# daxiongpro/EPNet

Hardware: AMD Instinct MI355X
Metric: SA-stack points/sec per GPU (16384-pt KITTI scene) + % HBM roofline (higher is better)
Workload: dtype f32; 1 GPU; 256 x 16384-pt kitti scenes per GPU per step through the 4-level SA op stack (4 samplings [FPS + centre gather; levels 2-4 nested in level 1 where tie-free] + 8 ball_query + 8 fused groupings [xyz - centre ; features]), pyramid 16384>4096>1024>256>64, radii [[.1,.5],[.5,1],[1,2],[2,4]], nsample [16,32], C=0/96/256/512, HIP-graph launch; levels=4, scenes_per_gpu=256, software_pipelined=True, pipeline_stages=2, parallelism=scene-parallel x1

## Files before the change

epnet_amd/csrc/group.hip:

```cpp

#include "common.h"
#include "spatial.h"
#include "runsum.h"

namespace epnet {

constexpr int kGThreads = 256;
constexpr int kGChan = 16;

__global__ __launch_bounds__(kGThreads) void gather_rows_vec4_kernel(int c, int n, int p, size_t ostride,
                                                                     const float *__restrict__ points,
                                                                     const int *__restrict__ idx,
                                                                     float *__restrict__ out) {
    int wg_x, wg_y, bs;
    xcd_scene_map3(wg_x, wg_y, bs);
    const int c0 = wg_y * kGChan;
    const int q4 = wg_x * kGThreads + threadIdx.x;
    if (q4 * 4 >= p) return;
    const int4 id = *reinterpret_cast<const int4 *>(idx + (size_t)bs * p + (size_t)q4 * 4);
    const int cend = min(c, c0 + kGChan);
    const float *src = points + ((size_t)bs * c + c0) * n;
    float *dst = out + (size_t)bs * ostride + (size_t)c0 * p + (size_t)q4 * 4;
#pragma unroll 4
    for (int ci = c0; ci < cend; ++ci) {
        float4 v;
        v.x = src[id.x];
        v.y = src[id.y];
        v.z = src[id.z];
        v.w = src[id.w];
        *reinterpret_cast<float4 *>(dst) = v;
        src += n;
        dst += p;
    }
}

__global__ __launch_bounds__(kGThreads) void gather_rows_scalar_kernel(int c, int n, int p, size_t ostride,
                                                                       const float *__restrict__ points,
                                                                       const int *__restrict__ idx,
                                                                       float *__restrict__ out) {
    int wg_x, wg_y, bs;
    xcd_scene_map3(wg_x, wg_y, bs);
    const int c0 = wg_y * kGChan;
    const int q = wg_x * kGThreads + threadIdx.x;
    if (q >= p) return;
    const int id = idx[(size_t)bs * p + q];
    const int cend = min(c, c0 + kGChan);
    for (int ci = c0; ci < cend; ++ci)
        out[(size_t)bs * ostride + (size_t)ci * p + q] = points[((size_t)bs * c + ci) * n + id];
}

#ifndef EPNET_GATHER_STAGE_UNROLL
#define EPNET_STAGE_PRAGMA
#else
#define EPNET_STAGE_STR2(x) #x
#define EPNET_STAGE_STR(x) EPNET_STAGE_STR2(unroll x)
#define EPNET_STAGE_PRAGMA _Pragma(EPNET_STAGE_STR(EPNET_GATHER_STAGE_UNROLL))
#endif
#ifndef EPNET_GATHER_LDS_BUDGET_KB
#define EPNET_GATHER_LDS_BUDGET_KB 64
#endif
#ifndef EPNET_GATHER_LDS_THREADS
#define EPNET_GATHER_LDS_THREADS 256
#endif
#ifndef EPNET_GATHER_LDS_UNROLL
#define EPNET_GATHER_LDS_UNROLL 1
#endif
constexpr int kGLdsThreads = EPNET_GATHER_LDS_THREADS;
__device__ __forceinline__ void stage_quads(const float *__restrict__ src, int groups, int n, float4 *__restrict__ s_quad,
                                            int threads) {
    const int n4 = n >> 2;
    for (int e = threadIdx.x; e < groups * n4; e += threads) {
        const int g = e / n4, j4 = e - g * n4;
        const float4 *row = reinterpret_cast<const float4 *>(src + (size_t)g * 4 * n) + j4;
        const float4 a = row[0], b4 = row[n4], cc = row[2 * n4], d = row[3 * n4];
        float4 *dst = s_quad + (size_t)g * n + j4 * 4;
        dst[0] = make_float4(a.x, b4.x, cc.x, d.x);
        dst[1] = make_float4(a.y, b4.y, cc.y, d.y);
        dst[2] = make_float4(a.z, b4.z, cc.z, d.z);
        dst[3] = make_float4(a.w, b4.w, cc.w, d.w);
    }
}

__device__ __forceinline__ void serve_quads(const float4 *__restrict__ quad, int groups, int n, int4 id, float *__restrict__ dst,
                                            int p) {
#pragma unroll 1
    for (int g = 0; g < groups; ++g) {
        const float4 v0 = quad[id.x], v1 = quad[id.y], v2 = quad[id.z], v3 = quad[id.w];
        store_stream(dst, v0.x, v1.x, v2.x, v3.x);
        store_stream(dst + p, v0.y, v1.y, v2.y, v3.y);
        store_stream(dst + 2 * (size_t)p, v0.z, v1.z, v2.z, v3.z);
        store_stream(dst + 3 * (size_t)p, v0.w, v1.w, v2.w, v3.w);
        quad += n;
        dst += 4 * (size_t)p;
    }
}

template <bool QUAD>
__global__ __launch_bounds__(kGLdsThreads) void gather_rows_lds_kernel(int c, int n, int p, int rows, int tile, size_t ostride,
                                                                    const float *__restrict__ points,
                                                                    const int *__restrict__ idx,
                                                                    float *__restrict__ out) {
    extern __shared__ float s_rows[];
    int wg_x, wg_y, bs;
    xcd_scene_map3(wg_x, wg_y, bs);
    const int c0 = wg_y * rows;
    const int nr = min(rows, c - c0);
    const float *src = points + ((size_t)bs * c + c0) * n;
    const int total = nr * n;
    if (QUAD) {
        stage_quads(src, nr >> 2, n, reinterpret_cast<float4 *>(s_rows), kGLdsThreads);
    } else if ((n & 3) == 0 && ((uintptr_t)src & 15) == 0) {
        const float4 *src4 = reinterpret_cast<const float4 *>(src);
        float4 *dst4 = reinterpret_cast<float4 *>(s_rows);
        EPNET_STAGE_PRAGMA
        for (int e = threadIdx.x; e < total / 4; e += kGLdsThreads) dst4[e] = src4[e];
    } else {
        for (int e = threadIdx.x; e < total; e += kGLdsThreads) s_rows[e] = src[e];
    }
    __syncthreads();
    const int q_begin = wg_x * tile, q_end = min(p, q_begin + tile);
    const int *ix = idx + (size_t)bs * p;
    float *dst_base = out + (size_t)bs * ostride + (size_t)c0 * p;
    for (int q = q_begin + threadIdx.x * 4; q < q_end; q += kGLdsThreads * 4) {
        const int4 id = *reinterpret_cast<const int4 *>(ix + q);
        float *dst = dst_base + q;
        if (QUAD) {
            serve_quads(reinterpret_cast<const float4 *>(s_rows), nr >> 2, n, id, dst, p);
            continue;
        }
        const float *row = s_rows;
#pragma unroll EPNET_GATHER_LDS_UNROLL
        for (int r = 0; r < nr; ++r) {
            float4 v;
            v.x = row[id.x];
            v.y = row[id.y];
            v.z = row[id.z];
            v.w = row[id.w];
            store_stream(dst, v.x, v.y, v.z, v.w);
            row += n;
            dst += p;
        }
    }
}

#ifndef EPNET_GATHER_LDS2_UNROLL
#define EPNET_GATHER_LDS2_UNROLL 1
#endif
constexpr long long kGatherLds2MinPositions = 3 * kGLdsThreads * 4;
template <bool QUAD>
__global__ __launch_bounds__(kGLdsThreads) void gather_rows_lds2_kernel(int c, int n, int rows, const float *__restrict__ points,
                                                                        int p0, size_t ostride0, const int *__restrict__ idx0,
                                                                        float *__restrict__ out0, int p1, size_t ostride1,
                                                                        const int *__restrict__ idx1, float *__restrict__ out1) {
    extern __shared__ float s_rows[];
    int wg_x, bs;
    xcd_scene_map(wg_x, bs);
    const int c0 = wg_x * rows;
    const int nr = min(rows, c - c0);
    const float *src = points + ((size_t)bs * c + c0) * n;
    const int total = nr * n;
    if (QUAD) {
        stage_quads(src, nr >> 2, n, reinterpret_cast<float4 *>(s_rows), kGLdsThreads);
    } else if ((n & 3) == 0 && ((uintptr_t)src & 15) == 0) {
        const float4 *src4 = reinterpret_cast<const float4 *>(src);
        float4 *dst4 = reinterpret_cast<float4 *>(s_rows);
        EPNET_STAGE_PRAGMA
        for (int e = threadIdx.x; e < total / 4; e += kGLdsThreads) dst4[e] = src4[e];
    } else {
        for (int e = threadIdx.x; e < total; e += kGLdsThreads) s_rows[e] = src[e];
    }
    __syncthreads();
#pragma unroll 1
    for (int set = 0; set < 2; ++set) {
        const int p = set ? p1 : p0;
        const int *ix = (set ? idx1 : idx0) + (size_t)bs * p;
        float *dst_base = (set ? out1 : out0) + (size_t)bs * (set ? ostride1 : ostride0) + (size_t)c0 * p;
        for (int q = threadIdx.x * 4; q < p; q += kGLdsThreads * 4) {
            const int4 id = *reinterpret_cast<const int4 *>(ix + q);
            float *dst = dst_base + q;
            if (QUAD) {
                serve_quads(reinterpret_cast<const float4 *>(s_rows), nr >> 2, n, id, dst, p);
                continue;
            }
            const float *row = s_rows;
#pragma unroll EPNET_GATHER_LDS2_UNROLL
            for (int r = 0; r < nr; ++r) {
                float4 v;
                v.x = row[id.x];
                v.y = row[id.y];
                v.z = row[id.z];
                v.w = row[id.w];
                store_stream(dst, v.x, v.y, v.z, v.w);
                row += n;
                dst += p;
            }
        }
    }
}

__global__ __launch_bounds__(kGThreads) void scatter_rows_lds_kernel(int c, int n, int p, int rows, size_t gstride,
                                                                     const float *__restrict__ grad_out,
                                                                     const int *__restrict__ idx,
                                                                     float *__restrict__ grad_points) {
    extern __shared__ float acc[];
    const int bs = blockIdx.y;
    const int c0 = blockIdx.x * rows;
    const int nr = min(rows, c - c0);
    for (int e = threadIdx.x; e < nr * n; e += kGThreads) acc[e] = 0.f;
    __syncthreads();
    const int *ix = idx + (size_t)bs * p;
    const float *go = grad_out + (size_t)bs * gstride + (size_t)c0 * p;
    for (int q = threadIdx.x; q < p; q += kGThreads) {
        const int id = ix[q];
        for (int r = 0; r < nr; ++r) atomicAdd(&acc[r * n + id], go[(size_t)r * p + q]);
    }
    __syncthreads();
    float *gp = grad_points + ((size_t)bs * c + c0) * n;
    for (int e = threadIdx.x; e < nr * n; e += kGThreads) gp[e] += acc[e];
}

__global__ __launch_bounds__(kGThreads) void scatter_rows_atomic_kernel(int c, int n, int p, size_t gstride,
                                                                        const float *__restrict__ grad_out,
                                                                        const int *__restrict__ idx,
                                                                        float *__restrict__ grad_points) {
    const int bs = blockIdx.z, ci = blockIdx.y;
    const int q = blockIdx.x * kGThreads + threadIdx.x;
    if (q >= p) return;
    atomicAdd(grad_points + ((size_t)bs * c + ci) * n + idx[(size_t)bs * p + q],
              grad_out[(size_t)bs * gstride + (size_t)ci * p + q]);
}

__global__ __launch_bounds__(kGThreads) void group_xyz_centred_kernel(int n, int npoints, int nsample, size_t ostride,
                                                                      const float *__restrict__ xyz,
                                                                      const float *__restrict__ new_xyz,
                                                                      const int *__restrict__ idx, float *__restrict__ out) {
    int wg_x, bs;
    xcd_scene_map(wg_x, bs);
    const int p = npoints * nsample;
    const int q = wg_x * kGThreads + threadIdx.x;
    if (q >= p) return;
    const int id = idx[(size_t)bs * p + q];
    const int ci = q / nsample;
    const float *pt = xyz + ((size_t)bs * n + id) * 3;
    const float *ce = new_xyz + ((size_t)bs * npoints + ci) * 3;
    float *dst = out + (size_t)bs * ostride + q;
    dst[0] = pt[0] - ce[0];
    dst[(size_t)p] = pt[1] - ce[1];
    dst[(size_t)p * 2] = pt[2] - ce[2];
}

__global__ __launch_bounds__(kGThreads) void group_xyz_centred_vec4_kernel(int n, int npoints, int nsample, size_t ostride,
                                                                           const float *__restrict__ xyz,
                                                                           const float *__restrict__ new_xyz,
                                                                           const int *__restrict__ idx,
                                                                           float *__restrict__ out) {
    int wg_x, bs;
    xcd_scene_map(wg_x, bs);
    const int p = npoints * nsample;
    const int q = (wg_x * kGThreads + threadIdx.x) * 4;
    if (q >= p) return;
    const int4 id = *reinterpret_cast<const int4 *>(idx + (size_t)bs * p + q);
    const float *base = xyz + (size_t)bs * n * 3;
    const float *ce = new_xyz + ((size_t)bs * npoints + q / nsample) * 3;
    const float cx = ce[0], cy = ce[1], cz = ce[2];
    const float *p0 = base + (size_t)id.x * 3, *p1 = base + (size_t)id.y * 3, *p2 = base + (size_t)id.z * 3,
                *p3 = base + (size_t)id.w * 3;
    float *dst = out + (size_t)bs * ostride + q;
    *reinterpret_cast<float4 *>(dst) = make_float4(p0[0] - cx, p1[0] - cx, p2[0] - cx, p3[0] - cx);
    *reinterpret_cast<float4 *>(dst + (size_t)p) = make_float4(p0[1] - cy, p1[1] - cy, p2[1] - cy, p3[1] - cy);
    *reinterpret_cast<float4 *>(dst + (size_t)p * 2) = make_float4(p0[2] - cz, p1[2] - cz, p2[2] - cz, p3[2] - cz);
}

__global__ __launch_bounds__(kGLdsThreads) void group_linear_lds_kernel(int c, int n, int npoints, int nsample, int rows, int tile,
                                                                        const float *__restrict__ z, const float *__restrict__ xyz,
                                                                        const float *__restrict__ new_xyz, const int *__restrict__ idx,
                                                                        const float *__restrict__ wx, const float *__restrict__ bias,
                                                                        float *__restrict__ out) {
    extern __shared__ float s_rows[];
    const int bs = blockIdx.z;
    const int c0 = blockIdx.y * rows;
    const int nr = min(rows, c - c0);
    const int p = npoints * nsample;
    const float *src = z + ((size_t)bs * c + c0) * n;
    const int total = nr * n;
    if ((n & 3) == 0 && ((uintptr_t)src & 15) == 0) {
        const float4 *src4 = reinterpret_cast<const float4 *>(src);
        float4 *dst4 = reinterpret_cast<float4 *>(s_rows);
        EPNET_STAGE_PRAGMA
        for (int e = threadIdx.x; e < total / 4; e += kGLdsThreads) dst4[e] = src4[e];
    } else {
        for (int e = threadIdx.x; e < total; e += kGLdsThreads) s_rows[e] = src[e];
    }
    __syncthreads();
    const int q_begin = blockIdx.x * tile, q_end = min(p, q_begin + tile);
    const int *ix = idx + (size_t)bs * p;
    const float *pts = xyz + (size_t)bs * n * 3;
    float *dst_base = out + ((size_t)bs * c + c0) * p;
    for (int q = q_begin + threadIdx.x * 4; q < q_end; q += kGLdsThreads * 4) {
        const int4 id = *reinterpret_cast<const int4 *>(ix + q);
        const float *ce = new_xyz + ((size_t)bs * npoints + q / nsample) * 3;
        const float cx = ce[0], cy = ce[1], cz = ce[2];
        const float *p0 = pts + (size_t)id.x * 3, *p1 = pts + (size_t)id.y * 3, *p2 = pts + (size_t)id.z * 3, *p3 = pts + (size_t)id.w * 3;
        const float dx0 = p0[0] - cx, dy0 = p0[1] - cy, dz0 = p0[2] - cz;
        const float dx1 = p1[0] - cx, dy1 = p1[1] - cy, dz1 = p1[2] - cz;
        const float dx2 = p2[0] - cx, dy2 = p2[1] - cy, dz2 = p2[2] - cz;
        const float dx3 = p3[0] - cx, dy3 = p3[1] - cy, dz3 = p3[2] - cz;
        float *dst = dst_base + q;
        const float *row = s_rows;
#pragma unroll 2
        for (int r = 0; r < nr; ++r) {
            const float w0 = wx[(c0 + r) * 3], w1 = wx[(c0 + r) * 3 + 1], w2 = wx[(c0 + r) * 3 + 2];
            float4 v;
            v.x = row[id.x] + (w0 * dx0 + w1 * dy0 + w2 * dz0);
            v.y = row[id.y] + (w0 * dx1 + w1 * dy1 + w2 * dz1);
            v.z = row[id.z] + (w0 * dx2 + w1 * dy2 + w2 * dz2);
            v.w = row[id.w] + (w0 * dx3 + w1 * dy3 + w2 * dz3);
            if (bias) {
                const float bv = bias[c0 + r];
                v.x += bv; v.y += bv; v.z += bv; v.w += bv;
            }
            store_stream(dst, v.x, v.y, v.z, v.w);
            row += n;
            dst += p;
        }
    }
}

__global__ __launch_bounds__(kGThreads) void group_linear_scalar_kernel(int c, int n, int npoints, int nsample,
                                                                        const float *__restrict__ z, const float *__restrict__ xyz,
                                                                        const float *__restrict__ new_xyz, const int *__restrict__ idx,
                                                                        const float *__restrict__ wx, const float *__restrict__ bias,
                                                                        float *__restrict__ out) {
    const int bs = blockIdx.z;
    const int c0 = blockIdx.y * kGChan;
    const int p = npoints * nsample;
    const int q = blockIdx.x * kGThreads + threadIdx.x;
    if (q >= p) return;
    const int id = idx[(size_t)bs * p + q];
    const float *pt = xyz + ((size_t)bs * n + id) * 3;
    const float *ce = new_xyz + ((size_t)bs * npoints + q / nsample) * 3;
    const float dx = pt[0] - ce[0], dy = pt[1] - ce[1], dz = pt[2] - ce[2];
    const int cend = min(c, c0 + kGChan);
    for (int ci = c0; ci < cend; ++ci) {
        float v = z[((size_t)bs * c + ci) * n + id] + (wx[ci * 3] * dx + wx[ci * 3 + 1] * dy + wx[ci * 3 + 2] * dz);
        if (bias) v += bias[ci];
        out[((size_t)bs * c + ci) * p + q] = v;
    }
}

constexpr int kGwRows = 8;
__global__ __launch_bounds__(kGThreads) void group_linear_grad_w_kernel(int c, int n, int npoints, int nsample, int tile,
                                                                        const float *__restrict__ grad_out,
                                                                        const float *__restrict__ xyz,
                                                                        const float *__restrict__ new_xyz,
                                                                        const int *__restrict__ idx, float *__restrict__ grad_w) {
    __shared__ float s_part[kGThreads / 64][kGwRows * 3];
    const int bs = blockIdx.z;
    const int c0 = blockIdx.y * kGwRows;
    const int nr = min(kGwRows, c - c0);
    const int p = npoints * nsample;
    const int q_begin = blockIdx.x * tile, q_end = min(p, q_begin + tile);
    const int *ix = idx + (size_t)bs * p;
    const float *pts = xyz + (size_t)bs * n * 3;
    const float *g = grad_out + ((size_t)bs * c + c0) * p;
    float acc[kGwRows][3];
#pragma unroll
    for (int r = 0; r < kGwRows; ++r) acc[r][0] = acc[r][1] = acc[r][2] = 0.f;
    for (int q = q_begin + threadIdx.x; q < q_end; q += kGThreads) {
        const int id = ix[q];
        const float *pt = pts + (size_t)id * 3;
        const float *ce = new_xyz + ((size_t)bs * npoints + q / nsample) * 3;
        float gv[kGwRows];
#pragma unroll
        for (int r = 0; r < kGwRows; ++r) gv[r] = g[(size_t)min(r, nr - 1) * p + q];
        const float dx = pt[0] - ce[0], dy = pt[1] - ce[1], dz = pt[2] - ce[2];
#pragma unroll
        for (int r = 0; r < kGwRows; ++r) {
            const float gr = r < nr ? gv[r] : 0.f;
            acc[r][0] += gr * dx;
            acc[r][1] += gr * dy;
            acc[r][2] += gr * dz;
        }
    }
    const int lane = lane_id(), wave = threadIdx.x >> 6;
#pragma unroll
    for (int r = 0; r < kGwRows; ++r)
#pragma unroll
        for (int k = 0; k < 3; ++k) {
            const float v = wave_sum_f32(acc[r][k]);
            if (lane == 0) s_part[wave][r * 3 + k] = v;
        }
    __syncthreads();
    if (threadIdx.x < nr * 3) {
        float v = 0.f;
#pragma unroll
        for (int w = 0; w < kGThreads / 64; ++w) v += s_part[w][threadIdx.x];
        atomicAdd(grad_w + (size_t)c0 * 3 + threadIdx.x, v);
    }
}

constexpr int kPmThreads = 256;
constexpr int kPmTile = 128;

__global__ __launch_bounds__(256) void transpose_cn_kernel(int c, int n, const float *__restrict__ src, float *__restrict__ dst) {
    __shared__ float tile[64][65];
    const int bs = blockIdx.z, n0 = blockIdx.x * 64, c0 = blockIdx.y * 64;
    src += (size_t)bs * c * n;
    dst += (size_t)bs * c * n;
    const int tx = threadIdx.x & 63, ty = threadIdx.x >> 6;
    for (int r = ty; r < 64; r += 4)
        if (c0 + r < c && n0 + tx < n) tile[r][tx] = src[(size_t)(c0 + r) * n + n0 + tx];
    __syncthreads();
    for (int r = ty; r < 64; r += 4)
        if (n0 + r < n && c0 + tx < c) dst[(size_t)(n0 + r) * c + c0 + tx] = tile[tx][r];
}

__device__ __forceinline__ int pm_slot(int ch, int r) { return ch * kPmTile + (r ^ (((ch >> 2) & 7) << 2)); }

__global__ __launch_bounds__(kPmThreads) void gather_rows_pm_kernel(int c, int n, int p, size_t ostride,
                                                                    const float *__restrict__ points_t,
                                                                    const int *__restrict__ idx, float *__restrict__ out) {
    extern __shared__ float s_tile[];
    int wg_x, bs;
    xcd_scene_map(wg_x, bs);
    const int q0 = wg_x * kPmTile;
    const int t = threadIdx.x, lane = t & 63, wave = t >> 6;
    const int lanes_per_row = c >> 2, rows_per_pass = kPmThreads / lanes_per_row;
    points_t += (size_t)bs * n * c;
    idx += (size_t)bs * p;
    out += (size_t)bs * ostride;
    const int cnt = min(kPmTile, p - q0);
    const int r_in = t / lanes_per_row, l_in = t - r_in * lanes_per_row;
    constexpr int kMaxPass = 8;
    if (r_in < rows_per_pass) {
        for (int r0 = r_in; r0 < cnt; r0 += rows_per_pass * kMaxPass) {
            int j[kMaxPass];
            float4 v[kMaxPass];
#pragma unroll
            for (int k = 0; k < kMaxPass; ++k) {
                const int r = r0 + k * rows_per_pass;
                j[k] = r < cnt ? idx[q0 + r] : 0;
            }
#pragma unroll
            for (int k = 0; k < kMaxPass; ++k) v[k] = reinterpret_cast<const float4 *>(points_t + (size_t)j[k] * c)[l_in];
#pragma unroll
            for (int k = 0; k < kMaxPass; ++k) {
                const int r = r0 + k * rows_per_pass;
                if (r < cnt) {
                    const int ch = l_in * 4;
                    float *d = s_tile + pm_slot(ch, r);
                    d[0] = v[k].x; d[kPmTile] = v[k].y; d[2 * kPmTile] = v[k].z; d[3 * kPmTile] = v[k].w;
                }
            }
        }
    }
    __syncthreads();
    const bool wide = cnt == kPmTile && (p & 3) == 0 && (((uintptr_t)out) & 15) == 0;
    if (wide) {
        const int half = lane >> 5, l = lane & 31;
        for (int ch = wave * 2 + half; ch < c; ch += (kPmThreads / 64) * 2) {
            const float4 v = *reinterpret_cast<const float4 *>(s_tile + pm_slot(ch, l * 4));
            store_stream(out + (size_t)ch * p + q0 + l * 4, v.x, v.y, v.z, v.w);
        }
    } else {
        for (int ch = wave; ch < c; ch += kPmThreads / 64) {
            float *dst = out + (size_t)ch * p + q0;
#pragma unroll
            for (int k = 0; k < kPmTile / 64; ++k) {
                const int r = k * 64 + lane;
                if (r < cnt) __builtin_nontemporal_store(s_tile[pm_slot(ch, r)], dst + r);
            }
        }
    }
}

static size_t gather_pm_ws_bytes(int b, int c, int n, long long p) {
    constexpr int kLdsBudget = EPNET_GATHER_LDS_BUDGET_KB * 1024;
    if (b <= 0 || c < 16 || c > 128 || (c & 3) || (size_t)n * 4 <= (size_t)kLdsBudget || p < (long long)n) return 0;
    return (size_t)b * c * n * sizeof(float);
}

static int launch_gather_rows_pm(int b, int c, int n, long long p, const float *points, const int *idx, float *out, size_t ostride,
                                 void *workspace, hipStream_t s, const char *what) {
    if (b > 65535 || p > 0x7fffffffll) return EPNET_ELIMIT;
    float *pt = (float *)workspace;
    int chunk = (int)((64ll << 20) / ((long long)c * n * 4));
    if (chunk < 1) chunk = 1;
    for (int b0 = 0; b0 < b; b0 += chunk) {
        const int nb = min(chunk, b - b0);
        const float *src = points + (size_t)b0 * c * n;
        float *dst = pt + (size_t)b0 * c * n;
        hipLaunchKernelGGL(transpose_cn_kernel, dim3(div_up(n, 64), div_up(c, 64), nb), dim3(256), 0, s, c, n, src, dst);
        int rc = check_launch("feature transpose");
        if (rc) return rc;
        hipLaunchKernelGGL(gather_rows_pm_kernel, dim3((unsigned)div_up64(p, kPmTile), nb), dim3(kPmThreads),
                           (size_t)kPmTile * c * sizeof(float), s, c, n, (int)p, ostride, dst, idx + (size_t)b0 * p,
                           out + (size_t)b0 * ostride);
        rc = check_launch(what);
        if (rc) return rc;
    }
    return EPNET_OK;
}

static int launch_gather_rows(int b, int c, int n, long long p, const float *points, const int *idx, float *out,
                              hipStream_t s, const char *what, size_t ostride = 0) {
    if (ostride == 0) ostride = (size_t)c * (size_t)p;
    if (b == 0 || c == 0 || p == 0) return EPNET_OK;
    if (!(points && idx && out)) return EPNET_EINVAL;
    if (n <= 0) return EPNET_EINVAL;
    if (p > 0x7fffffffll || b > 65535 || div_up(c, kGChan) > 65535) return EPNET_ELIMIT;
    const bool vec = (p % 4 == 0) && (((uintptr_t)idx | (uintptr_t)out) % 16 == 0);
    constexpr int kLdsBudget = EPNET_GATHER_LDS_BUDGET_KB * 1024;
    if (vec && c >= 8 && (size_t)n * 4 <= kLdsBudget && p >= 2048) {
        int rows = kLdsBudget / (n * 4);
        if (rows > c) rows = c;
        if (rows > 32) rows = 32;
        const bool quad = (c & 3) == 0 && (n & 3) == 0 && rows >= 4 && ((uintptr_t)points & 15) == 0;
        if (quad) rows &= ~3;
        const int chunks = div_up(c, rows);
        int tiles = div_up(1024, b * chunks);
        const int max_tiles = (int)(p / 2048);
        if (tiles > max_tiles) tiles = max_tiles;
        if (tiles < 1) tiles = 1;
        int tile = (int)div_up64(p, tiles);
        tile = (tile + kGLdsThreads * 4 - 1) / (kGLdsThreads * 4) * (kGLdsThreads * 4);
        tiles = (int)div_up64(p, tile);
        if (chunks <= 65535) {
            dim3 grid(tiles, chunks, b);
            if (quad)
                hipLaunchKernelGGL(gather_rows_lds_kernel<true>, grid, dim3(kGLdsThreads), (size_t)rows * n * 4, s, c, n, (int)p, rows,
                                   tile, ostride, points, idx, out);
            else
                hipLaunchKernelGGL(gather_rows_lds_kernel<false>, grid, dim3(kGLdsThreads), (size_t)rows * n * 4, s, c, n, (int)p, rows,
                                   tile, ostride, points, idx, out);
            return check_launch(what);
        }
    }
    if (vec) {
        dim3 grid((unsigned)div_up64(p / 4, kGThreads), div_up(c, kGChan), b);
        hipLaunchKernelGGL(gather_rows_vec4_kernel, grid, dim3(kGThreads), 0, s, c, n, (int)p, ostride, points, idx, out);
    } else {
        dim3 grid((unsigned)div_up64(p, kGThreads), div_up(c, kGChan), b);
        hipLaunchKernelGGL(gather_rows_scalar_kernel, grid, dim3(kGThreads), 0, s, c, n, (int)p, ostride, points, idx, out);
    }
    return check_launch(what);
}

static size_t scatter_ws_bytes(int b, int n, long long p) {
    if (b <= 0 || !runsum::usable(n, 1, p, p)) return 0;
    return runsum::workspace_bytes(b, n, 1, p, false);
}

static int launch_scatter_rows_csr(int b, int c, int n, long long p, const float *grad_out, const int *idx,
                                   float *grad_points, void *workspace, size_t workspace_bytes, hipStream_t s,
                                   const char *what, size_t gstride) {
    if (gstride == 0) gstride = (size_t)c * (size_t)p;
    if (b == 0 || c == 0 || p == 0 || n == 0) return EPNET_OK;
    if (!(grad_out && idx && grad_points && workspace)) return EPNET_EINVAL;
    return runsum::launch<false>(b, c, n, 1, (int)p, grad_out, gstride, idx, nullptr, grad_points, workspace, workspace_bytes, s,
                                 what);
}

static int launch_scatter_rows(int b, int c, int n, long long p, const float *grad_out, const int *idx,
                               float *grad_points, hipStream_t s, const char *what, size_t gstride = 0) {
    if (gstride == 0) gstride = (size_t)c * (size_t)p;
    if (b == 0 || c == 0 || p == 0 || n == 0) return EPNET_OK;
    if (!(grad_out && idx && grad_points)) return EPNET_EINVAL;
    if (p > 0x7fffffffll || b > 65535) return EPNET_ELIMIT;
    constexpr int kLdsBudget = EPNET_GATHER_LDS_BUDGET_KB * 1024;
    if ((size_t)n * 4 <= kLdsBudget) {
        int rows = kLdsBudget / (n * 4);
        if (rows > 8) rows = 8;
        if (rows > c) rows = c;
        dim3 grid(div_up(c, rows), b);
        hipLaunchKernelGGL(scatter_rows_lds_kernel, grid, dim3(kGThreads), (size_t)rows * n * 4, s, c, n, (int)p, rows, gstride,
                           grad_out, idx, grad_points);
    } else {
        if (c > 65535) return EPNET_ELIMIT;
        dim3 grid((unsigned)div_up64(p, kGThreads), c, b);
        hipLaunchKernelGGL(scatter_rows_atomic_kernel, grid, dim3(kGThreads), 0, s, c, n, (int)p, gstride, grad_out, idx,
                           grad_points);
    }
    return check_launch(what);
}

}

using namespace epnet;

extern "C" int epnet_gather_points(int b, int c, int n, int npoints, const float *points, const int *idx, float *out,
                                   epnet_stream_t stream) {
    EPNET_REQUIRE(b >= 0 && c >= 0 && n >= 0 && npoints >= 0);
    return launch_gather_rows(b, c, n, npoints, points, idx, out, (hipStream_t)stream, "gather_points");
}

extern "C" int epnet_gather_points_grad(int b, int c, int n, int npoints, const float *grad_out, const int *idx,
                                        float *grad_points, epnet_stream_t stream) {
    EPNET_REQUIRE(b >= 0 && c >= 0 && n >= 0 && npoints >= 0);
    return launch_scatter_rows(b, c, n, npoints, grad_out, idx, grad_points, (hipStream_t)stream, "gather_points_grad");
}

extern "C" int epnet_group_points(int b, int c, int n, int npoints, int nsample, const float *points, const int *idx,
                                  float *out, epnet_stream_t stream) {
    EPNET_REQUIRE(b >= 0 && c >= 0 && n >= 0 && npoints >= 0 && nsample >= 0);
    return launch_gather_rows(b, c, n, (long long)npoints * nsample, points, idx, out, (hipStream_t)stream,
                              "group_points");
}

extern "C" int epnet_group_points_grad(int b, int c, int n, int npoints, int nsample, const float *grad_out,
                                       const int *idx, float *grad_points, epnet_stream_t stream) {
    EPNET_REQUIRE(b >= 0 && c >= 0 && n >= 0 && npoints >= 0 && nsample >= 0);
    return launch_scatter_rows(b, c, n, (long long)npoints * nsample, grad_out, idx, grad_points, (hipStream_t)stream,
                               "group_points_grad");
}

static int launch_group_xyz(int b, int n, int npoints, int nsample, long long p, size_t ostride, const float *xyz,
                            const float *new_xyz, const int *idx, float *out, hipStream_t s) {
    if (nsample % 4 == 0 && (((uintptr_t)idx | (uintptr_t)out) % 16 == 0) && (ostride % 4 == 0))
        hipLaunchKernelGGL(group_xyz_centred_vec4_kernel, dim3((unsigned)div_up64(p / 4, kGThreads), b), dim3(kGThreads), 0, s, n,
                           npoints, nsample, ostride, xyz, new_xyz, idx, out);
    else
        hipLaunchKernelGGL(group_xyz_centred_kernel, dim3((unsigned)div_up64(p, kGThreads), b), dim3(kGThreads), 0, s, n, npoints,
                           nsample, ostride, xyz, new_xyz, idx, out);
    return check_launch("group_concat xyz");
}

extern "C" int epnet_group_concat(int b, int c, int n, int npoints, int nsample, const float *xyz, const float *new_xyz,
                                  const float *features, const int *idx, float *out, int use_xyz, epnet_stream_t stream) {
    EPNET_REQUIRE(b >= 0 && c >= 0 && n >= 0 && npoints >= 0 && nsample >= 0);
    EPNET_REQUIRE(use_xyz || c > 0);
    const long long p = (long long)npoints * nsample;
    if (b == 0 || p == 0) return EPNET_OK;
    EPNET_REQUIRE(idx && out && (c == 0 || features) && (!use_xyz || (xyz && new_xyz)));
    EPNET_REQUIRE(n > 0);
    if (p > 0x7fffffffll || b > 65535) return EPNET_ELIMIT;
    hipStream_t s = (hipStream_t)stream;
    const int ch0 = use_xyz ? 3 : 0;
    const size_t ostride = (size_t)(ch0 + c) * (size_t)p;
    if (use_xyz) {
        int rc = launch_group_xyz(b, n, npoints, nsample, p, ostride, xyz, new_xyz, idx, out, s);
        if (rc) return rc;
    }
    if (c == 0) return EPNET_OK;
    return launch_gather_rows(b, c, n, p, features, idx, out + (size_t)ch0 * p, s, "group_concat features", ostride);
}

extern "C" size_t epnet_group_concat_workspace_bytes(int b, int c, int n, int npoints, int nsample) {
    return gather_pm_ws_bytes(b, c, n, (long long)npoints * nsample);
}

extern "C" int epnet_group_concat_ws(int b, int c, int n, int npoints, int nsample, const float *xyz, const float *new_xyz,
                                     const float *features, const int *idx, float *out, int use_xyz, void *workspace,
                                     size_t workspace_bytes, epnet_stream_t stream) {
    const long long p = (long long)npoints * nsample;
    const size_t need = gather_pm_ws_bytes(b, c, n, p);
    if (need == 0 || !workspace || ((uintptr_t)workspace & 15))
        return epnet_group_concat(b, c, n, npoints, nsample, xyz, new_xyz, features, idx, out, use_xyz, stream);
    if (workspace_bytes < need) return EPNET_ENOMEM;
    EPNET_REQUIRE(b >= 0 && n > 0 && npoints >= 0 && nsample >= 0 && features && idx && out && (!use_xyz || (xyz && new_xyz)));
    if (p > 0x7fffffffll || b > 65535) return EPNET_ELIMIT;
    const int ch0 = use_xyz ? 3 : 0;
    const size_t ostride = (size_t)(ch0 + c) * (size_t)p;
    if (use_xyz) {
        int rc = launch_group_xyz(b, n, npoints, nsample, p, ostride, xyz, new_xyz, idx, out, (hipStream_t)stream);
        if (rc) return rc;
    }
    return launch_gather_rows_pm(b, c, n, p, features, idx, out + (size_t)ch0 * p, ostride, workspace, (hipStream_t)stream,
                                 "group_concat features");
}

extern "C" int epnet_group_concat_multi(int b, int c, int n, int npoints, int nscales, const int *nsamples, const float *xyz,
                                        const float *new_xyz, const float *features, const int *const *idx, float *const *out,
                                        int use_xyz, epnet_stream_t stream) {
    EPNET_REQUIRE(nscales >= 0 && (nscales == 0 || (nsamples && idx && out)));
    hipStream_t s = (hipStream_t)stream;
    const int ch0 = use_xyz ? 3 : 0;
    constexpr int kLdsBudget = EPNET_GATHER_LDS_BUDGET_KB * 1024;
    bool fused = nscales == 2 && c >= 8 && b > 0 && n > 0 && npoints > 0 && (size_t)n * 4 <= (size_t)kLdsBudget && features && b <= 65535;
    int rows = 0;
    bool quad = false;
    if (fused) {
        rows = kLdsBudget / (n * 4);
        if (rows > c) rows = c;
        if (rows > 32) rows = 32;
        quad = (c & 3) == 0 && (n & 3) == 0 && rows >= 4 && ((uintptr_t)features & 15) == 0;
        if (quad) rows &= ~3;
        long long p_both = 0;
        for (int k = 0; k < 2 && fused; ++k) {
            const long long p = (long long)npoints * nsamples[k];
            fused = p > 0 && p <= 0x7fffffffll && p % 4 == 0 && idx[k] && out[k] &&
                    (((uintptr_t)idx[k] | (uintptr_t)out[k]) % 16 == 0) && ((size_t)(ch0 + c) * (size_t)p) % 4 == 0;
            p_both += p;
        }
        fused = fused && p_both >= kGatherLds2MinPositions;
        fused = fused && (long long)b * div_up(c, rows) >= 512;
    }
    if (!fused) {
        for (int k = 0; k < nscales; ++k) {
            const int rc = epnet_group_concat(b, c, n, npoints, nsamples[k], xyz, new_xyz, features, idx[k], out[k], use_xyz, stream);
            if (rc) return rc;
        }
        return EPNET_OK;
    }
    size_t ostride[2];
    int pk[2];
    for (int k = 0; k < 2; ++k) {
        pk[k] = npoints * nsamples[k];
        ostride[k] = (size_t)(ch0 + c) * (size_t)pk[k];
        if (!use_xyz) continue;
        EPNET_REQUIRE(xyz && new_xyz);
        const long long p = pk[k];
        if (nsamples[k] % 4 == 0)
            hipLaunchKernelGGL(group_xyz_centred_vec4_kernel, dim3((unsigned)div_up64(p / 4, kGThreads), b), dim3(kGThreads), 0, s,
                               n, npoints, nsamples[k], ostride[k], xyz, new_xyz, idx[k], out[k]);
        else
            hipLaunchKernelGGL(group_xyz_centred_kernel, dim3((unsigned)div_up64(p, kGThreads), b), dim3(kGThreads), 0, s, n,
                               npoints, nsamples[k], ostride[k], xyz, new_xyz, idx[k], out[k]);
        const int rc = check_launch("group_concat_multi xyz");
        if (rc) return rc;
    }
    if (quad)
        hipLaunchKernelGGL(gather_rows_lds2_kernel<true>, dim3(div_up(c, rows), b), dim3(kGLdsThreads), (size_t)rows * n * 4, s, c, n,
                           rows, features, pk[0], ostride[0], idx[0], out[0] + (size_t)ch0 * pk[0], pk[1], ostride[1], idx[1],
                           out[1] + (size_t)ch0 * pk[1]);
    else
        hipLaunchKernelGGL(gather_rows_lds2_kernel<false>, dim3(div_up(c, rows), b), dim3(kGLdsThreads), (size_t)rows * n * 4, s, c, n,
                           rows, features, pk[0], ostride[0], idx[0], out[0] + (size_t)ch0 * pk[0], pk[1], ostride[1], idx[1],
                           out[1] + (size_t)ch0 * pk[1]);
    return check_launch("group_concat_multi");
}

extern "C" int epnet_group_concat_grad(int b, int c, int n, int npoints, int nsample, const float *grad_out, const int *idx,
                                       float *grad_features, int use_xyz, epnet_stream_t stream) {
    EPNET_REQUIRE(b >= 0 && c >= 0 && n >= 0 && npoints >= 0 && nsample >= 0);
    const long long p = (long long)npoints * nsample;
    if (b == 0 || c == 0 || p == 0) return EPNET_OK;
    const int ch0 = use_xyz ? 3 : 0;
    const size_t gstride = (size_t)(ch0 + c) * (size_t)p;
    return launch_scatter_rows(b, c, n, p, grad_out + (size_t)ch0 * p, idx, grad_features, (hipStream_t)stream,
                               "group_concat_grad", gstride);
}

extern "C" size_t epnet_group_points_grad_workspace_bytes(int b, int n, int npoints, int nsample) {
    return scatter_ws_bytes(b, n, (long long)npoints * nsample);
}

extern "C" int epnet_group_points_grad_ws(int b, int c, int n, int npoints, int nsample, const float *grad_out,
                                          const int *idx, float *grad_points, void *workspace, size_t workspace_bytes,
                                          epnet_stream_t stream) {
    EPNET_REQUIRE(b >= 0 && c >= 0 && n >= 0 && npoints >= 0 && nsample >= 0);
    const long long p = (long long)npoints * nsample;
    if (scatter_ws_bytes(b, n, p) == 0 || ((uintptr_t)grad_out & 15))
        return launch_scatter_rows(b, c, n, p, grad_out, idx, grad_points, (hipStream_t)stream, "group_points_grad");
    return launch_scatter_rows_csr(b, c, n, p, grad_out, idx, grad_points, workspace, workspace_bytes, (hipStream_t)stream,
                                   "group_points_grad", 0);
}

extern "C" int epnet_group_concat_grad_ws(int b, int c, int n, int npoints, int nsample, const float *grad_out,
                                          const int *idx, float *grad_features, int use_xyz, void *workspace,
                                          size_t workspace_bytes, epnet_stream_t stream) {
    EPNET_REQUIRE(b >= 0 && c >= 0 && n >= 0 && npoints >= 0 && nsample >= 0);
    const long long p = (long long)npoints * nsample;
    if (b == 0 || c == 0 || p == 0) return EPNET_OK;
    const int ch0 = use_xyz ? 3 : 0;
    const size_t gstride = (size_t)(ch0 + c) * (size_t)p;
    if (scatter_ws_bytes(b, n, p) == 0 || ((uintptr_t)grad_out & 15))
        return launch_scatter_rows(b, c, n, p, grad_out + (size_t)ch0 * p, idx, grad_features, (hipStream_t)stream,
                                   "group_concat_grad", gstride);
    return launch_scatter_rows_csr(b, c, n, p, grad_out + (size_t)ch0 * p, idx, grad_features, workspace, workspace_bytes,
                                   (hipStream_t)stream, "group_concat_grad", gstride);
}

extern "C" int epnet_group_linear(int b, int c, int n, int npoints, int nsample, const float *xyz, const float *new_xyz,
                                  const float *z, const int *idx, const float *w_xyz, const float *bias, float *out,
                                  epnet_stream_t stream) {
    EPNET_REQUIRE(b >= 0 && c >= 0 && n >= 0 && npoints >= 0 && nsample >= 0);
    const long long p = (long long)npoints * nsample;
    if (b == 0 || c == 0 || p == 0) return EPNET_OK;
    EPNET_REQUIRE(xyz && new_xyz && z && idx && w_xyz && out && n > 0);
    if (p > 0x7fffffffll || b > 65535 || div_up(c, kGChan) > 65535) return EPNET_ELIMIT;
    hipStream_t s = (hipStream_t)stream;
    constexpr int kLdsBudget = EPNET_GATHER_LDS_BUDGET_KB * 1024;
    const bool vec = nsample % 4 == 0 && (((uintptr_t)idx | (uintptr_t)out) % 16 == 0);
    if (vec && c >= 8 && (size_t)n * 4 <= (size_t)kLdsBudget && p >= 1024) {
        int rows = kLdsBudget / (n * 4);
        if (rows > c) rows = c;
        if (rows > 32) rows = 32;
        const int chunks = div_up(c, rows);
        int tiles = div_up(1024, b * chunks);
        const int max_tiles = (int)(p / 1024);
        if (tiles > max_tiles) tiles = max_tiles;
        if (tiles < 1) tiles = 1;
        int tile = (int)div_up64(p, tiles);
        tile = (tile + kGLdsThreads * 4 - 1) / (kGLdsThreads * 4) * (kGLdsThreads * 4);
        tiles = (int)div_up64(p, tile);
        if (chunks <= 65535) {
            hipLaunchKernelGGL(group_linear_lds_kernel, dim3(tiles, chunks, b), dim3(kGLdsThreads), (size_t)rows * n * 4, s, c, n, npoints,
                               nsample, rows, tile, z, xyz, new_xyz, idx, w_xyz, bias, out);
            return check_launch("group_linear");
        }
    }
    hipLaunchKernelGGL(group_linear_scalar_kernel, dim3((unsigned)div_up64(p, kGThreads), div_up(c, kGChan), b), dim3(kGThreads), 0, s, c,
                       n, npoints, nsample, z, xyz, new_xyz, idx, w_xyz, bias, out);
    return check_launch("group_linear");
}

extern "C" int epnet_group_linear_grad_w(int b, int c, int n, int npoints, int nsample, const float *grad_out, const float *xyz,
                                         const float *new_xyz, const int *idx, float *grad_w, epnet_stream_t stream) {
    EPNET_REQUIRE(b >= 0 && c >= 0 && n >= 0 && npoints >= 0 && nsample >= 0);
    const long long p = (long long)npoints * nsample;
    if (b == 0 || c == 0 || p == 0) return EPNET_OK;
    EPNET_REQUIRE(grad_out && xyz && new_xyz && idx && grad_w && n > 0);
    const int chunks = div_up(c, kGwRows);
    if (p > 0x7fffffffll || b > 65535 || chunks > 65535) return EPNET_ELIMIT;
    int tiles = div_up(2048, b * chunks);
    const int max_tiles = (int)div_up64(p, 1024);
    if (tiles > max_tiles) tiles = max_tiles;
    if (tiles < 1) tiles = 1;
    const int tile = (int)div_up64(p, tiles);
    tiles = (int)div_up64(p, tile);
    hipLaunchKernelGGL(group_linear_grad_w_kernel, dim3(tiles, chunks, b), dim3(kGThreads), 0, (hipStream_t)stream, c, n, npoints,
                       nsample, tile, grad_out, xyz, new_xyz, idx, grad_w);
    return check_launch("group_linear_grad_w");
}
```

Baseline: 1.435 billion points/s.

## Software-pipeline index loads and specialize quad LDS gather by group count

Rewrites the quad-transposed LDS gather path. Index int4 loads are now prefetched one trip ahead and double-buffered, and the first index load is issued before the LDS-stage barrier. The per-thread loop is templated on the number of 4-row groups with a switch dispatch, and staging is unrolled 2x with incremental unsigned byte offsets. The aim is to hide global index-load latency and cut address arithmetic, in exchange for more register pressure, code size, and sched_barrier constraints.

```diff
diff --git a/epnet_amd/csrc/group.hip b/epnet_amd/csrc/group.hip
--- a/epnet_amd/csrc/group.hip
+++ b/epnet_amd/csrc/group.hip
@@ -66,34 +66,159 @@
 #define EPNET_GATHER_LDS_UNROLL 1
 #endif
 constexpr int kGLdsThreads = EPNET_GATHER_LDS_THREADS;
+__device__ __forceinline__ void stage_quad_store(float4 *__restrict__ dst, float4 a, float4 b4, float4 cc, float4 d) {
+    dst[0] = make_float4(a.x, b4.x, cc.x, d.x);
+    dst[1] = make_float4(a.y, b4.y, cc.y, d.y);
+    dst[2] = make_float4(a.z, b4.z, cc.z, d.z);
+    dst[3] = make_float4(a.w, b4.w, cc.w, d.w);
+}
+
+template <typename T>
+__device__ __forceinline__ T *byte_at(T *base, unsigned bytes) {
+    typedef typename std::conditional<std::is_const<T>::value, const char, char>::type byte_t;
+    return reinterpret_cast<T *>(reinterpret_cast<byte_t *>(base) + bytes);
+}
+
 __device__ __forceinline__ void stage_quads(const float *__restrict__ src, int groups, int n, float4 *__restrict__ s_quad,
                                             int threads) {
-    const int n4 = n >> 2;
-    for (int e = threadIdx.x; e < groups * n4; e += threads) {
-        const int g = e / n4, j4 = e - g * n4;
-        const float4 *row = reinterpret_cast<const float4 *>(src + (size_t)g * 4 * n) + j4;
-        const float4 a = row[0], b4 = row[n4], cc = row[2 * n4], d = row[3 * n4];
-        float4 *dst = s_quad + (size_t)g * n + j4 * 4;
-        dst[0] = make_float4(a.x, b4.x, cc.x, d.x);
-        dst[1] = make_float4(a.y, b4.y, cc.y, d.y);
-        dst[2] = make_float4(a.z, b4.z, cc.z, d.z);
-        dst[3] = make_float4(a.w, b4.w, cc.w, d.w);
-    }
-}
-
+    const unsigned n4 = (unsigned)n >> 2, total = groups * n4, step = threads;
+    const float4 *r0 = reinterpret_cast<const float4 *>(src), *r1 = r0 + n4, *r2 = r1 + n4, *r3 = r2 + n4;
+    const unsigned dg = step / n4, dj = step - dg * n4;
+    unsigned e = threadIdx.x, g = e / n4, j = e - g * n4;
+    for (; e + step < total; e += 2 * step) {
+        unsigned g1 = g + dg, j1 = j + dj;
+        if (j1 >= n4) j1 -= n4, ++g1;
+        const unsigned o0 = (g * n + j) * 16u, o1 = (g1 * n + j1) * 16u;
+        const float4 a0 = *byte_at(r0, o0), b0 = *byte_at(r1, o0), c0 = *byte_at(r2, o0), d0 = *byte_at(r3, o0);
+        const float4 a1 = *byte_at(r0, o1), b1 = *byte_at(r1, o1), c1 = *byte_at(r2, o1), d1 = *byte_at(r3, o1);
+        stage_quad_store(byte_at(s_quad, (g * n + j * 4) * 16u), a0, b0, c0, d0);
+        stage_quad_store(byte_at(s_quad, (g1 * n + j1 * 4) * 16u), a1, b1, c1, d1);
+        g = g1 + dg, j = j1 + dj;
+        if (j >= n4) j -= n4, ++g;
+    }
+    if (e < total) {
+        const unsigned o = (g * n + j) * 16u;
+        const float4 a = *byte_at(r0, o), b4 = *byte_at(r1, o), cc = *byte_at(r2, o), d = *byte_at(r3, o);
+        stage_quad_store(byte_at(s_quad, (g * n + j * 4) * 16u), a, b4, cc, d);
+    }
+}
+
+__device__ __forceinline__ void serve_quad_group(const float4 *__restrict__ quad, int4 id, float *__restrict__ dst, unsigned tb, int p) {
+    asm volatile("" : "+v"(tb));
+    const float4 v0 = quad[id.x], v1 = quad[id.y], v2 = quad[id.z], v3 = quad[id.w];
+    store_stream(byte_at(dst, tb), v0.x, v1.x, v2.x, v3.x);
+    store_stream(byte_at(dst + p, tb), v0.y, v1.y, v2.y, v3.y);
+    store_stream(byte_at(dst + 2 * (size_t)p, tb), v0.z, v1.z, v2.z, v3.z);
+    store_stream(byte_at(dst + 3 * (size_t)p, tb), v0.w, v1.w, v2.w, v3.w);
+}
+
+template <int G>
 __device__ __forceinline__ void serve_quads(const float4 *__restrict__ quad, int groups, int n, int4 id, float *__restrict__ dst,
-                                            int p) {
+                                            unsigned tb, int p) {
+    if constexpr (G > 0) {
+#pragma unroll
+        for (int g = 0; g < G; ++g) {
+            serve_quad_group(quad, id, dst, tb, p);
+            __builtin_amdgcn_sched_barrier(0);
+            quad += n;
+            dst += 4 * (size_t)p;
+        }
+    } else {
 #pragma unroll 1
-    for (int g = 0; g < groups; ++g) {
-        const float4 v0 = quad[id.x], v1 = quad[id.y], v2 = quad[id.z], v3 = quad[id.w];
-        store_stream(dst, v0.x, v1.x, v2.x, v3.x);
-        store_stream(dst + p, v0.y, v1.y, v2.y, v3.y);
-        store_stream(dst + 2 * (size_t)p, v0.z, v1.z, v2.z, v3.z);
-        store_stream(dst + 3 * (size_t)p, v0.w, v1.w, v2.w, v3.w);
-        quad += n;
-        dst += 4 * (size_t)p;
-    }
-}
+        for (int g = 0; g < groups; ++g) {
+            serve_quad_group(quad, id, dst, tb, p);
+            quad += n;
+            dst += 4 * (size_t)p;
+        }
+    }
+}
+
+constexpr unsigned kGPass = kGLdsThreads * 4;
+
+template <int K>
+__device__ __forceinline__ void load_index_quads(int4 (&id)[K], const int *__restrict__ ix, unsigned q, unsigned q_last, unsigned t4) {
+#pragma unroll
+    for (int k = 0; k < K; ++k) {
+        const unsigned base = min(q + k * kGPass, q_last);
+        id[k] = *reinterpret_cast<const int4 *>(byte_at(ix + base, min(t4, q_last - base) * 4u));
+    }
+}
+
+template <int G, int K>
+__device__ __forceinline__ void serve_trip(const float4 *__restrict__ quad, int groups, int n, const int4 (&id)[K],
+                                           float *__restrict__ dst_base, int p, unsigned q, unsigned t4) {
+#pragma unroll
+    for (int k = 0; k < K; ++k) serve_quads<G>(quad, groups, n, id[k], dst_base + (q + k * kGPass), t4 * 4u, p);
+}
+
+template <int G, int K, bool NEXT>
+__device__ __forceinline__ void serve_span(const float4 *__restrict__ quad, int groups, int n, const int *__restrict__ ix,
+                                           float *__restrict__ dst_base, int p, unsigned q_begin, unsigned q_end, int4 (&a)[K],
+                                           const int *__restrict__ ix_next, unsigned nq_begin, unsigned nq_last) {
+    constexpr unsigned kTrip = K * kGPass;
+    const unsigned q_last = q_end - 4, t4 = threadIdx.x * 4;
+    unsigned q = q_begin;
+    unsigned full = (q_end - q_begin) / kTrip;
+    int4 b[K];
+    auto two_trips = [&]() {
+        load_index_quads<K>(b, ix, q + kTrip, q_last, t4);
+        serve_trip<G, K>(quad, groups, n, a, dst_base, p, q, t4);
+        load_index_quads<K>(a, ix, q + 2 * kTrip, q_last, t4);
+        serve_trip<G, K>(quad, groups, n, b, dst_base, p, q + kTrip, t4);
+        q += 2 * kTrip;
+        full -= 2;
+    };
+    if (full >= 2) {
+        two_trips();
+#pragma unroll 1
+        while (full >= 2) two_trips();
+    }
+    if (full) {
+        serve_trip<G, K>(quad, groups, n, a, dst_base, p, q, t4);
+        q += kTrip;
+    }
+    if (NEXT) load_index_quads<K>(a, ix_next, nq_begin, nq_last, t4);
+#pragma unroll 1
+    for (; q < q_end; q += kGPass) {
+        if (q + t4 >= q_end) continue;
+        const int4 id = *reinterpret_cast<const int4 *>(byte_at(ix + q, t4 * 4u));
+        serve_quads<G>(quad, groups, n, id, dst_base + q, t4 * 4u, p);
+    }
+}
+
+template <int G, int K>
+__device__ __forceinline__ void gather_rows_lds_quad(const float *__restrict__ src, int groups, int n, int p, const int *__restrict__ ix,
+                                                     float *__restrict__ dst_base, unsigned q_begin, unsigned q_end) {
+    extern __shared__ float s_rows[];
+    int4 a[K];
+    stage_quads(src, groups, n, reinterpret_cast<float4 *>(s_rows), kGLdsThreads);
+    load_index_quads<K>(a, ix, q_begin, q_end - 4, threadIdx.x * 4);
+    __syncthreads();
+    serve_span<G, K, false>(reinterpret_cast<const float4 *>(s_rows), groups, n, ix, dst_base, p, q_begin, q_end, a, nullptr, 0, 0);
+}
+
+template <int G, int K>
+__device__ __forceinline__ void gather_rows_lds2_quad(const float *__restrict__ src, int groups, int n, int p0, const int *__restrict__ ix0,
+                                                      float *__restrict__ dst0, int p1, const int *__restrict__ ix1,
+                                                      float *__restrict__ dst1) {
+    extern __shared__ float s_rows[];
+    int4 a[K];
+    stage_quads(src, groups, n, reinterpret_cast<float4 *>(s_rows), kGLdsThreads);
+    load_index_quads<K>(a, ix0, 0, p0 - 4, threadIdx.x * 4);
+    __syncthreads();
+    const float4 *quad = reinterpret_cast<const float4 *>(s_rows);
+    serve_span<G, K, true>(quad, groups, n, ix0, dst0, p0, 0, p0, a, ix1, 0, p1 - 4);
+    serve_span<G, K, false>(quad, groups, n, ix1, dst1, p1, 0, p1, a, nullptr, 0, 0);
+}
+
+#define EPNET_GATHER_QUAD_DISPATCH(groups, FN, ...)            \
+    switch (groups) {                                          \
+        case 1: FN<1, 4>(__VA_ARGS__); break;                  \
+        case 2: FN<2, 2>(__VA_ARGS__); break;                  \
+        case 4: FN<4, 1>(__VA_ARGS__); break;                  \
+        case 8: FN<8, 1>(__VA_ARGS__); break;                  \
+        default: FN<0, 1>(__VA_ARGS__); break;                 \
+    }
 
 template <bool QUAD>
 __global__ __launch_bounds__(kGLdsThreads) void gather_rows_lds_kernel(int c, int n, int p, int rows, int tile, size_t ostride,
@@ -106,10 +231,15 @@
     const int c0 = wg_y * rows;
     const int nr = min(rows, c - c0);
     const float *src = points + ((size_t)bs * c + c0) * n;
+    const int q_begin = wg_x * tile, q_end = min(p, q_begin + tile);
+    const int *ix = idx + (size_t)bs * p;
+    float *dst_base = out + (size_t)bs * ostride + (size_t)c0 * p;
+    if (QUAD) {
+        EPNET_GATHER_QUAD_DISPATCH(nr >> 2, gather_rows_lds_quad, src, nr >> 2, n, p, ix, dst_base, (unsigned)q_begin, (unsigned)q_end)
+        return;
+    }
     const int total = nr * n;
-    if (QUAD) {
-        stage_quads(src, nr >> 2, n, reinterpret_cast<float4 *>(s_rows), kGLdsThreads);
-    } else if ((n & 3) == 0 && ((uintptr_t)src & 15) == 0) {
+    if ((n & 3) == 0 && ((uintptr_t)src & 15) == 0) {
         const float4 *src4 = reinterpret_cast<const float4 *>(src);
         float4 *dst4 = reinterpret_cast<float4 *>(s_rows);
         EPNET_STAGE_PRAGMA
@@ -118,16 +248,9 @@
         for (int e = threadIdx.x; e < total; e += kGLdsThreads) s_rows[e] = src[e];
     }
     __syncthreads();
-    const int q_begin = wg_x * tile, q_end = min(p, q_begin + tile);
-    const int *ix = idx + (size_t)bs * p;
-    float *dst_base = out + (size_t)bs * ostride + (size_t)c0 * p;
     for (int q = q_begin + threadIdx.x * 4; q < q_end; q += kGLdsThreads * 4) {
         const int4 id = *reinterpret_cast<const int4 *>(ix + q);
         float *dst = dst_base + q;
-        if (QUAD) {
-            serve_quads(reinterpret_cast<const float4 *>(s_rows), nr >> 2, n, id, dst, p);
-            continue;
-        }
         const float *row = s_rows;
 #pragma unroll EPNET_GATHER_LDS_UNROLL
         for (int r = 0; r < nr; ++r) {
@@ -158,10 +281,14 @@
     const int c0 = wg_x * rows;
     const int nr = min(rows, c - c0);
     const float *src = points + ((size_t)bs * c + c0) * n;
+    if (QUAD) {
+        EPNET_GATHER_QUAD_DISPATCH(nr >> 2, gather_rows_lds2_quad, src, nr >> 2, n, p0, idx0 + (size_t)bs * p0,
+                                   out0 + (size_t)bs * ostride0 + (size_t)c0 * p0, p1, idx1 + (size_t)bs * p1,
+                                   out1 + (size_t)bs * ostride1 + (size_t)c0 * p1)
+        return;
+    }
     const int total = nr * n;
-    if (QUAD) {
-        stage_quads(src, nr >> 2, n, reinterpret_cast<float4 *>(s_rows), kGLdsThreads);
-    } else if ((n & 3) == 0 && ((uintptr_t)src & 15) == 0) {
+    if ((n & 3) == 0 && ((uintptr_t)src & 15) == 0) {
         const float4 *src4 = reinterpret_cast<const float4 *>(src);
         float4 *dst4 = reinterpret_cast<float4 *>(s_rows);
         EPNET_STAGE_PRAGMA
@@ -178,10 +305,6 @@
         for (int q = threadIdx.x * 4; q < p; q += kGLdsThreads * 4) {
             const int4 id = *reinterpret_cast<const int4 *>(ix + q);
             float *dst = dst_base + q;
-            if (QUAD) {
-                serve_quads(reinterpret_cast<const float4 *>(s_rows), nr >> 2, n, id, dst, p);
-                continue;
-            }
             const float *row = s_rows;
 #pragma unroll EPNET_GATHER_LDS2_UNROLL
             for (int r = 0; r < nr; ++r) {
```

Result: no change. 1.437 billion points/s, median of 2 (+0.2%).
